# coecms/xmhw

Measured on AMD Instinct MI355X. Metric: grid-cells/sec for threshold() on 40yr daily SST, higher is better.
Workload: dtype f32 in / f64 out; 1 GPU; 0.25deg global (configs[2]): 1036800 cells per step, 1982-2021 (T=14610), windowHalfWidth=5, pctile=90, smoothPercentileWidth=31, nan_frac=0.0, skipna=False; cells_rank0=1036800, T=14610, D=366, kernel=clim_sorted_f32 (sorted row-lists in LDS, 2 lanes per cell, layout 40), slabs=1, gather=none

## Files before the change

xmhw_amd/csrc/kernels_sorted.hip:

```cpp
#include <type_traits>

#include "device_common.h"
#include "kernels.h"
#include "packed_src.h"
#include "plan.h"
#include "sortnet_gen.h"

namespace xmhw {
namespace {

typedef __attribute__((address_space(3))) uint32_t lds_u32;
__device__ __forceinline__ uint32_t lds_ld(uint32_t a) { return *reinterpret_cast<lds_u32*>(static_cast<uintptr_t>(a)); }
__device__ __forceinline__ void lds_st(uint32_t a, uint32_t v) { *reinterpret_cast<lds_u32*>(static_cast<uintptr_t>(a)) = v; }

constexpr int kSwap1 = 0xB1;
__device__ __forceinline__ uint32_t swp(uint32_t v) {
    return static_cast<uint32_t>(__builtin_amdgcn_update_dpp(0, static_cast<int>(v), kSwap1, 0xF, 0xF, true));
}
__device__ __forceinline__ double swp(double v) {
    const uint64_t b = static_cast<uint64_t>(__double_as_longlong(v));
    const uint32_t lo = swp(static_cast<uint32_t>(b)), hi = swp(static_cast<uint32_t>(b >> 32));
    return __longlong_as_double(static_cast<long long>((static_cast<uint64_t>(hi) << 32) | lo));
}
__device__ __forceinline__ uint32_t med3u(uint32_t a, uint32_t b, uint32_t c) {
    uint32_t r;
    asm("v_med3_u32 %0, %1, %2, %3" : "=v"(r) : "v"(a), "v"(b), "v"(c));
    return r;
}
__device__ __forceinline__ bool wave_any(bool c) { return __builtin_amdgcn_ballot_w64(c) != 0ull; }
__device__ __forceinline__ uint32_t mad_u24(uint32_t a, uint32_t b, uint32_t c) {
    uint32_t r;
    asm("v_mad_u32_u24 %0, %1, %2, %3" : "=v"(r) : "v"(a), "s"(b), "v"(c));
    return r;
}
__device__ __forceinline__ uint32_t mad_i24(uint32_t a, int32_t b, uint32_t c) {
    uint32_t r;
    asm("v_mad_i32_i24 %0, %1, %2, %3" : "=v"(r) : "v"(a), "v"(b), "v"(c));
    return r;
}
__device__ __forceinline__ uint32_t umin(uint32_t a, uint32_t b) { return a < b ? a : b; }
__device__ __forceinline__ uint32_t umax(uint32_t a, uint32_t b) { return a > b ? a : b; }

template <bool NEG>
__device__ __forceinline__ uint32_t key_fast(uint32_t b) {
    const int32_t sg = static_cast<int32_t>(b) >> 31;
    if constexpr (NEG)
        return static_cast<uint32_t>(__builtin_amdgcn_bitop3_b32(sg, static_cast<int32_t>(b), static_cast<int32_t>(0x80000000u), 0xC9));
    else
        return static_cast<uint32_t>(__builtin_amdgcn_bitop3_b32(sg, static_cast<int32_t>(b), static_cast<int32_t>(0x80000000u), 0x36));
}

__device__ __forceinline__ uint32_t count_ge4(uint32_t a0, uint32_t a1, uint32_t a2, uint32_t a3, uint32_t th) {
    uint32_t c;
    unsigned long long s0, s1, s2, s3, sd;
    asm("v_cmp_ge_u32_e64 %[s0], %[a0], %[t]\n\t"
        "v_cmp_ge_u32_e64 %[s1], %[a1], %[t]\n\t"
        "v_cmp_ge_u32_e64 %[s2], %[a2], %[t]\n\t"
        "v_cmp_ge_u32_e64 %[s3], %[a3], %[t]\n\t"
        "v_addc_co_u32_e64 %[c], %[sd], 0, 0, %[s0]\n\t"
        "v_addc_co_u32_e64 %[c], %[sd], %[c], 0, %[s1]\n\t"
        "v_addc_co_u32_e64 %[c], %[sd], %[c], 0, %[s2]\n\t"
        "v_addc_co_u32_e64 %[c], %[sd], %[c], 0, %[s3]"
        : [c] "=&v"(c), [s0] "=&s"(s0), [s1] "=&s"(s1), [s2] "=&s"(s2), [s3] "=&s"(s3), [sd] "=&s"(sd)
        : [a0] "v"(a0), [a1] "v"(a1), [a2] "v"(a2), [a3] "v"(a3), [t] "v"(th));
    return c;
}

typedef uint32_t V32 __attribute__((ext_vector_type(32)));
#ifdef XMHW_NO_COLD
#define XMHW_COLD(x) (x)
#else
#define XMHW_COLD(x) __builtin_expect(!!(x), 0)
#endif
#define XMHW_STR2(x) #x
#define XMHW_STR(x) XMHW_STR2(x)
#ifndef XMHW_LOOP_PAD
#define XMHW_LOOP_PAD 0
#endif

template <int N>
__device__ __forceinline__ void sort_desc(uint32_t (&v)[N]) {
    if constexpr (N >= 3 && N <= 7) {
        sortnet::Ins<N>::run(v);
    } else if constexpr (N == 8 || N == 10 || N == 12) {
        constexpr int H = N / 2;
        uint32_t a[H], b[H];
#pragma unroll
        for (int i = 0; i < H; ++i) { a[i] = v[i]; b[i] = v[H + i]; }
        sortnet::Ins<H>::run(a);
        sortnet::Ins<H>::run(b);
#pragma unroll
        for (int i = 0; i < H; ++i) { v[i] = a[i]; v[H + i] = b[i]; }
        sortnet::MergeTop<H, H, N>::run(v);
    } else {
        sortnet::Desc<N>::run(v);
    }
}
constexpr int kLdsGranule = 1280;


__device__ __forceinline__ uint32_t wave_min_u32(uint32_t v) {
    v = umin(v, static_cast<uint32_t>(__builtin_amdgcn_update_dpp(-1, static_cast<int>(v), 0xB1, 0xF, 0xF, false)));
    v = umin(v, static_cast<uint32_t>(__builtin_amdgcn_update_dpp(-1, static_cast<int>(v), 0x4E, 0xF, 0xF, false)));
    v = umin(v, static_cast<uint32_t>(__builtin_amdgcn_update_dpp(-1, static_cast<int>(v), 0x141, 0xF, 0xF, false)));
    v = umin(v, static_cast<uint32_t>(__builtin_amdgcn_update_dpp(-1, static_cast<int>(v), 0x140, 0xF, 0xF, false)));
    const uint32_t a = static_cast<uint32_t>(__builtin_amdgcn_readlane(static_cast<int>(v), 0));
    const uint32_t b = static_cast<uint32_t>(__builtin_amdgcn_readlane(static_cast<int>(v), 16));
    const uint32_t c = static_cast<uint32_t>(__builtin_amdgcn_readlane(static_cast<int>(v), 32));
    const uint32_t d = static_cast<uint32_t>(__builtin_amdgcn_readlane(static_cast<int>(v), 48));
    return umin(umin(a, b), umin(c, d));
}
__device__ __forceinline__ uint32_t wave_max_u32(uint32_t v) { return ~wave_min_u32(~v); }

template <int KPL>
__device__ __forceinline__ void pool_order_stats(const uint32_t (&key)[KPL], uint32_t n, uint32_t lo, uint32_t guess,
                                                 uint32_t& out_lo, uint32_t& out_hi) {
    auto count_lt = [&](uint32_t v) -> uint32_t {
        uint32_t cnt = 0;
#pragma unroll
        for (int i = 0; i < KPL; ++i)
            cnt += static_cast<uint32_t>(__builtin_popcountll(__builtin_amdgcn_ballot_w64(key[i] != 0u && key[i] < v)));
        return cnt;
    };
    auto count_eq = [&](uint32_t v) -> uint32_t {
        uint32_t cnt = 0;
#pragma unroll
        for (int i = 0; i < KPL; ++i)
            cnt += static_cast<uint32_t>(__builtin_popcountll(__builtin_amdgcn_ballot_w64(key[i] == v)));
        return cnt;
    };
    auto next_above = [&](uint32_t v) -> uint32_t {
        uint32_t m = 0xFFFFFFFFu;
#pragma unroll
        for (int i = 0; i < KPL; ++i) m = (key[i] > v && key[i] < m) ? key[i] : m;
        return wave_min_u32(m);
    };
    auto next_below = [&](uint32_t v) -> uint32_t {
        uint32_t m = 0;
#pragma unroll
        for (int i = 0; i < KPL; ++i) m = (key[i] < v && key[i] > m) ? key[i] : m;
        return wave_max_u32(m);
    };
    uint32_t v = guess;
    bool found = false;
    uint32_t cl = 0, ev = 0;
    if (v != 0u) {
        cl = count_lt(v);
        ev = count_eq(v);
        for (int it = 0; it < 32 && !found; ++it) {
            if (cl <= lo && lo < cl + ev) {
                found = true;
            } else if (lo < cl) {
                v = next_below(v);
                if (v == 0u) break;
                ev = count_eq(v);
                cl -= ev;
            } else {
                const uint32_t nv = next_above(v);
                if (nv == 0xFFFFFFFFu) break;
                cl += ev;
                v = nv;
                ev = count_eq(v);
            }
        }
    }
    if (!found) {
        v = 0;
        for (int bit = 31; bit >= 0; --bit) {
            const uint32_t cand = v | (1u << bit);
            uint32_t cnt = 0;
#pragma unroll
            for (int i = 0; i < KPL; ++i)
                cnt += static_cast<uint32_t>(__builtin_popcountll(__builtin_amdgcn_ballot_w64(key[i] - 1u < cand - 1u)));
            if (cnt <= lo) v = cand;
        }
        cl = count_lt(v);
        ev = count_eq(v);
    }
    uint32_t vhi = v;
    if (lo + 1 < n && lo + 1 >= cl + ev) vhi = next_above(v);
    out_lo = v;
    out_hi = vhi;
}

}

template <int YPS, int K, int KL, bool STATS, bool PACKED>
__device__ __forceinline__ void sorted_body(
    const void* __restrict__ ts, int64_t C, int64_t ld, int64_t Tn, const uint32_t* __restrict__ table,
    const uint32_t* __restrict__ sflags, const DevSortedChunk* __restrict__ chunks, double q, int negate,
    int32_t ntracks, double* __restrict__ thresh, double* __restrict__ seas, int64_t ldo,
    unsigned long long* __restrict__ stats, const PackedI16& pk) {
    constexpr int R = 11;
    constexpr uint32_t ES = PACKED ? 2u : 4u;
    constexpr int NL = 6;
    constexpr int HE = (YPS + 1) / 2 * 2;
    constexpr int HH = HE / 2;
    constexpr int KH = K / 2;
#ifndef XMHW_SERIAL_MAX
#define XMHW_SERIAL_MAX 3
#endif
    constexpr uint32_t kSerialMax = XMHW_SERIAL_MAX;
    constexpr int NTP = 2 * YPS;
    constexpr uint32_t LSTRIDE = 32 * 4;
    constexpr uint32_t RSTRIDE = R * LSTRIDE;
    constexpr int LDS_BYTES = (R * KL * static_cast<int>(LSTRIDE) + kLdsGranule - 1) / kLdsGranule * kLdsGranule;
    static_assert(K <= HE && K % 2 == 0, "a list stores an even number of keys, at most what a lane holds");
    constexpr int EXT = K - KL;
    static_assert(EXT == 0 || ((EXT == 2 || EXT == 4) && KL >= KH), "two or four register ranks, all from lane 1's half");
    constexpr int EXN = EXT > 0 ? EXT : 1;
    static_assert(LDS_BYTES == 8960 || LDS_BYTES == 11520 || LDS_BYTES == 14080 || LDS_BYTES == 17920 || LDS_BYTES == 20480 ||
                  LDS_BYTES == 23040 || LDS_BYTES == 25600, "sorted_lds_probe() checks these allocation sizes");
    __shared__ __attribute__((aligned(16))) uint32_t lds[LDS_BYTES / 4];

    const int lane = threadIdx.x & 63;
    const int sub = lane & 1;
    const int cw = lane >> 1;
    const int64_t cell = static_cast<int64_t>(blockIdx.x) * 32 + cw;
    const bool cell_ok = cell < C;
    const DevSortedChunk ch = chunks[blockIdx.y];
    const int32_t step_min = ch.warm_start - ch.trow0;
    const char* col = static_cast<const char*>(ts) + (cell_ok ? cell : C - 1) * static_cast<int64_t>(ES);
    const bool mirror = q < 0.5;
    const int kneg = (negate != 0) != mirror ? 1 : 0;
    const uint32_t tmax = static_cast<uint32_t>(Tn - 1);
    const bool padded_last = (YPS - 1) * 2 + sub >= ntracks;
    const uint32_t padmask = padded_last ? 0xFFFFFFFFu : 0u;
    const uint32_t* tab = table + sub;

    const uint32_t lds0 = static_cast<uint32_t>(reinterpret_cast<uintptr_t>((lds_u32*)lds));
    if (lds0 != 0u) __builtin_trap();
    const uint32_t lcell = static_cast<uint32_t>(cw) * 4u;
    for (int i = lane; i < LDS_BYTES / 4; i += 64) lds[i] = 0u;
    __builtin_amdgcn_s_waitcnt(0);
    __builtin_amdgcn_wave_barrier();

    uint32_t P[NL];
    V32 TV = 0;
#define XMHW_RSLO(j) TV[2 * (j)]
#define XMHW_RSHI(j) TV[2 * (j) + 1]
#define XMHW_EX(e, j) TV[12 + 6 * (e) + (j)]
#define XMHW_NVL(j) TV[24 + (j)]
    uint32_t lbase[NL];
#pragma unroll
    for (int j = 0; j < NL; ++j) {
        const int g = sub * NL + j;
        lbase[j] = g < R ? lcell + static_cast<uint32_t>(g) * LSTRIDE : 0x40000000u + lcell;
        P[j] = 0;
    }
    static_assert(KL >= 5, "a list holds a window");
    static_assert(NL == 6 && EXT <= 2, "the register vector holds five values of six lists");
#ifdef XMHW_WARM_SELECT
    uint32_t Ctop = 0, n = 0, B = 0u;
#else
    uint32_t Ctop = 0, n = 0, B = 0xFFFFFFFFu;
#endif
    double total = 0.0;

    const uint32_t ld4 = static_cast<uint32_t>(ld) * ES;
    const char* ap[YPS];
    auto entries_of = [&](int32_t step, uint32_t (&e)[YPS]) {
        const uint32_t* p = tab + static_cast<int64_t>(step - step_min) * NTP;
#pragma unroll
        for (int y = 0; y < YPS; ++y) e[y] = p[y * 2];
    };
    auto point_at = [&](int32_t step) {
        uint32_t e[YPS];
        entries_of(step, e);
#pragma unroll
        for (int y = 0; y < YPS; ++y) {
            const uint32_t t = umin((e[y] >> 1) - 2u, tmax);
            ap[y] = col + static_cast<uint64_t>(t) * ld4;
        }
    };
    auto advance = [&]() {
#pragma unroll
        for (int y = 0; y < YPS; ++y) ap[y] += (y == YPS - 1 && padded_last) ? 0u : ld4;
    };
    typename std::conditional<PACKED, int32_t, float>::type x_in[YPS];
    auto request = [&]() {
#pragma unroll
        for (int y = 0; y < YPS; ++y) {
            if constexpr (PACKED) x_in[y] = static_cast<int32_t>(*reinterpret_cast<const int16_t*>(ap[y]));
            else x_in[y] = *reinterpret_cast<const float*>(ap[y]);
        }
    };
    point_at(ch.warm_start);
    request();

    unsigned long long tacc[8] = {0, 0, 0, 0, 0, 0, 0, 0};
    unsigned long long tlast = 0;
    if constexpr (STATS) tlast = __builtin_amdgcn_s_memtime();
    auto tick = [&](int idx) {
        if constexpr (STATS) {
            __builtin_amdgcn_sched_barrier(0);
            asm volatile("s_waitcnt lgkmcnt(0)" ::: "memory");
            const unsigned long long now = __builtin_amdgcn_s_memtime();
            tacc[idx] += now - tlast;
            tlast = now;
            __builtin_amdgcn_sched_barrier(0);
        }
    };
    uint32_t st_rows = 0, st_iter = 0, st_flag = 0, st_steps = 0;
    uint32_t st_serial = 0, st_ext = 0;
    uint32_t st_more[4] = {0, 0, 0, 0};

    uint32_t e_alo = 0, e_ahi = 0, e_n = 0;
    double e_total = 0.0, e_g = 0.0;

    int32_t ep_s = -1;
    uint32_t ep_eph = 0;
    auto finish_rows = [&]() {
        double th = make_nan(), se = make_nan();
        if (e_n > 0) {
            double v_lo = static_cast<double>(key_f32(e_alo));
            double v_hi = static_cast<double>(key_f32(e_ahi));
            if (mirror) {
                v_lo = -v_lo;
                v_hi = -v_hi;
            }
            se = e_total / static_cast<double>(e_n);
            if constexpr (PACKED) {
                v_lo = packed_value(pk, v_lo);
                v_hi = packed_value(pk, v_hi);
                se = packed_value(pk, se);
            }
            th = numpy_lerp(v_lo, v_hi, e_g);
        }
        if (static_cast<uint32_t>(sub) <= ep_eph && cell_ok) {
            const int64_t row = static_cast<int64_t>(ep_s) - static_cast<int64_t>(ep_eph) + sub;
            thresh[row * ldo + cell] = th;
            seas[row * ldo + cell] = se;
        }
        ep_s = -1;
    };
    bool nan_mode = false;
    uint32_t vi_n = 0xFFFFFFFFu, vi_lo = 0;
    double vi_g = 0.0;
    int m = ((ch.warm_start % R) + R) % R;
    uint32_t sf_cur = __builtin_amdgcn_readfirstlane(sflags[ch.warm_start - step_min]);
    uint32_t sf_nxt = ch.warm_start + 1 < ch.end ? __builtin_amdgcn_readfirstlane(sflags[ch.warm_start + 1 - step_min]) : 0u;
#ifdef XMHW_LOOP_ALIGN
    asm volatile(".p2align " XMHW_STR(XMHW_LOOP_ALIGN) "\n\t.rept " XMHW_STR(XMHW_LOOP_PAD) "\n\ts_nop 0\n\t.endr" ::: "memory");
#endif
    for (int32_t s = ch.warm_start; s < ch.end; ++s) {
        const uint32_t sf = sf_cur;
        const uint32_t sf_nn = s + 2 < ch.end ? sflags[s + 2 - step_min] : 0u;
        uint32_t k[HE];
        double din = 0.0;
        uint32_t nvin = 0;
        float xv[YPS];
        bool packed_fill = false;
        if constexpr (STATS) {
            asm volatile("s_waitcnt vmcnt(0)" ::: "memory");
            tick(5);
        }
        if constexpr (PACKED) {
            if (pk.swap) {
#pragma unroll
                for (int y = 0; y < YPS; ++y)
                    x_in[y] = static_cast<int32_t>(static_cast<int16_t>(__builtin_bswap16(static_cast<uint16_t>(x_in[y]))));
            }
#pragma unroll
            for (int y = 0; y < YPS; ++y) xv[y] = static_cast<float>(x_in[y]);
            if (pk.mode == 1) {
#pragma unroll
                for (int y = 0; y < YPS; ++y) {
                    float f = xv[y] * pk.sf;
                    f = f + pk.of;
                    xv[y] = f;
                }
            }
            bool anyfill = false;
#pragma unroll
            for (int y = 0; y < YPS; ++y) anyfill = anyfill || x_in[y] == pk.fill;
            packed_fill = wave_any(anyfill);
            if (packed_fill) {
#pragma unroll
                for (int y = 0; y < YPS; ++y) xv[y] = x_in[y] == pk.fill ? __uint_as_float(0x7FC00000u) : xv[y];
            }
        } else {
#pragma unroll
            for (int y = 0; y < YPS; ++y) xv[y] = x_in[y];
        }
        bool slow = !(sf & 1u) || nan_mode;
        if (!slow) {
            auto plain_row = [&](auto negc, auto sumc) {
                constexpr bool NEG = decltype(negc)::value, SUM = decltype(sumc)::value;
                double din1 = 0.0;
#pragma unroll
                for (int y = 0; y < YPS; ++y) {
                    uint32_t xb = __float_as_uint(xv[y]);
                    uint32_t ky = key_fast<NEG>(xb);
                    if (y == YPS - 1) {
                        xb &= ~padmask;
                        ky &= ~padmask;
                    }
                    k[y] = ky;
                    if constexpr (SUM) {
                        const double dv = static_cast<double>(__uint_as_float(xb));
                        if (y & 1) din1 = y == 1 ? dv : din1 + dv;
                        else din = y == 0 ? dv : din + dv;
                    }
                }
                if constexpr (SUM) din += din1;
            };
            bool int_sum = false;
            if constexpr (PACKED) int_sum = pk.mode != 1;
            if (int_sum) {
                if constexpr (PACKED) {
                    int32_t isum = 0;
#pragma unroll
                    for (int y = 0; y < YPS; ++y)
                        isum += (y == YPS - 1) ? (x_in[y] & static_cast<int32_t>(~padmask)) : x_in[y];
                    if (kneg) plain_row(std::true_type{}, std::false_type{});
                    else plain_row(std::false_type{}, std::false_type{});
                    din = packed_fill ? make_nan() : static_cast<double>(isum);
                }
            } else if (kneg) {
                plain_row(std::true_type{}, std::true_type{});
            } else {
                plain_row(std::false_type{}, std::true_type{});
            }
            if (negate) din = -din;
            nvin = padded_last ? YPS - 1 : YPS;
            slow = wave_any(din != din);
            nan_mode = slow;
        }
        if (XMHW_COLD(slow)) {
            din = 0.0;
            nvin = 0;
#define XMHW_GENERAL_ROW(NEG_, OKEXPR)                                                                  \
    _Pragma("unroll") for (int y = 0; y < YPS; ++y) {                                                   \
        const float xs = xv[y];                                                                          \
        const bool ok = xs == xs && (OKEXPR);                                                            \
        k[y] = ok ? key_fast<NEG_>(__float_as_uint(xs)) : 0u;                                            \
        din += static_cast<double>(ok ? xs : 0.0f);                                                      \
        nvin += ok ? 1u : 0u;                                                                            \
    }
            if (sf & 1u) {
                if (kneg) { XMHW_GENERAL_ROW(true, !(y == YPS - 1 && padded_last)) }
                else { XMHW_GENERAL_ROW(false, !(y == YPS - 1 && padded_last)) }
            } else {
                uint32_t e[YPS];
                entries_of(s, e);
                if (kneg) { XMHW_GENERAL_ROW(true, (e[y] >> 1) >= 2u) }
                else { XMHW_GENERAL_ROW(false, (e[y] >> 1) >= 2u) }
            }
#undef XMHW_GENERAL_ROW
            if (negate) din = -din;
            if (sf & 1u) nan_mode = wave_any(nvin != static_cast<uint32_t>(padded_last ? YPS - 1 : YPS));
        }
#pragma unroll
        for (int y = YPS; y < HE; ++y) k[y] = 0u;
        tick(6);
        if (ep_s >= 0) finish_rows();
        if (s + 1 < ch.end) {
            if (!XMHW_COLD(!(sf_nxt & 2u))) advance();
            else point_at(s + 1);
            request();
        }
        tick(0);

        uint32_t u[KH];
        {
            uint32_t ka[HE];
            {
                uint32_t h0[HH], h1[HH];
#pragma unroll
                for (int i = 0; i < HH; ++i) { h0[i] = k[i]; h1[i] = k[HH + i]; }
                sort_desc<HH>(h0);
                sort_desc<HH>(h1);
#pragma unroll
                for (int i = 0; i < HH; ++i) { ka[i] = h0[i]; ka[HH + i] = h1[i]; }
            }
            sortnet::MergeTop<HH, HH, K>::run(ka);
            uint32_t t[K];
#pragma unroll
            for (int i = 0; i < K; ++i) t[i] = umax(ka[i], swp(ka[K - 1 - i]));
            const uint32_t lb = sub ? 0u : 0xFFFFFFFFu;
#pragma unroll
            for (int i = 0; i < KH; ++i) u[i] = med3u(t[i], t[i + KH], lb);
            sortnet::BitonicDesc<KH>::run(u);
        }
        tick(1);

        const int m_sub = m >= NL ? 1 : 0;
        const int mj = __builtin_amdgcn_readfirstlane(m - m_sub * NL);
        const bool own_m = sub == m_sub;
        const uint32_t base_m = lcell + static_cast<uint32_t>(m) * LSTRIDE + static_cast<uint32_t>(sub * KH) * RSTRIDE;
#pragma unroll
        for (int i = 0; i < KH; ++i) {
            if (EXT == 0 || i < KH - EXT || sub == 0) lds_st(base_m + static_cast<uint32_t>(i) * RSTRIDE, u[i]);
        }
        uint32_t c_old = 0, nv_old = 0;
        bool is_slot[NL];
#pragma unroll
        for (int j = 0; j < NL; ++j) {
            int mj_ = mj;
            asm volatile("" : "+s"(mj_));
            is_slot[j] = mj_ == j;
        }
        const uint32_t nvm = TV[24 + mj];
        {
            uint32_t Pm = P[0];
#pragma unroll
            for (int j = 1; j < NL; ++j) Pm = is_slot[j] ? P[j] : Pm;
            if (own_m) {
                c_old = Pm;
                nv_old = nvm;
            }
        }
        uint32_t c_new = 0;
#pragma unroll
        for (int i = 0; i < KH; ++i) c_new += (u[i] > B) ? 1u : 0u;
        {
            uint32_t pk = (c_new << 16) | nvin;
            uint32_t po = (c_old << 16) | nv_old;
            pk += swp(pk);
            po += swp(po);
            c_new = umin(pk >> 16, static_cast<uint32_t>(KL));
            nvin = pk & 0xFFFFu;
            c_old = po >> 16;
            nv_old = po & 0xFFFFu;
        }
        din += swp(din);
        Ctop += c_new - c_old;
        n += nvin - nv_old;
#pragma unroll
        for (int j = 0; j < NL; ++j) P[j] = (own_m && is_slot[j]) ? c_new : P[j];
        TV[24 + mj] = own_m ? nvin : nvm;
        if constexpr (EXT > 0) {
#pragma unroll
            for (int e_ = 0; e_ < EXT; ++e_) {
                const uint32_t r_ = swp(u[KH - EXT + e_]);
                const uint32_t mine = sub ? u[KH - EXT + e_] : r_;
                const uint32_t old_ = TV[12 + 6 * e_ + mj];
                TV[12 + 6 * e_ + mj] = own_m ? mine : old_;
            }
        }
        {
            const uint64_t db = static_cast<uint64_t>(__double_as_longlong(din));
            const uint32_t ol_ = TV[2 * mj], oh_ = TV[2 * mj + 1];
            TV[2 * mj] = own_m ? static_cast<uint32_t>(db) : ol_;
            TV[2 * mj + 1] = own_m ? static_cast<uint32_t>(db >> 32) : oh_;
        }
        {
            double tsum = 0.0;
#pragma unroll
            for (int j = 0; j < NL; ++j)
                tsum += __longlong_as_double(static_cast<long long>((static_cast<uint64_t>(XMHW_RSHI(j)) << 32) | XMHW_RSLO(j)));
            total = tsum + swp(tsum);
        }
        m = (m + 1 == R) ? 0 : m + 1;
        tick(2);

        uint32_t a_lo = 0, a_hi = 0;
        double g = 0.0;
        bool flag = false;
#ifdef XMHW_WARM_SELECT
        if (true) {
#else
        if (s >= ch.begin) {
#endif
        if (XMHW_COLD(wave_any(n != vi_n))) {
            vi_n = n;
            const uint32_t nn_ = n ? n : 1u;
            const double vi = static_cast<double>(nn_ - 1) * q;
            const double fl = floor(vi);
            vi_g = vi - fl;
            vi_lo = static_cast<uint32_t>(fl);
        }
        const uint32_t nn = n ? n : 1u;
        g = vi_g;
        const uint32_t lo = vi_lo;
        const bool need2 = lo + 1 < nn;
        const uint32_t Cs = n ? (mirror ? lo + 1u : n - 1u - lo) : 0u;
        const bool grow = Ctop <= Cs;
        uint32_t rem = grow ? Cs - Ctop : Ctop - Cs;
        const uint32_t steps0 = rem;
        const uint32_t cm = grow ? 0u : 0xFFFFFFFFu;
        const uint32_t cneg = grow ? 0u : 1u;
        auto cpl = [&](uint32_t v) -> uint32_t { return (v ^ cm) + cneg; };
        const int psign = grow ? 1 : -1;
        const int32_t dstep = grow ? static_cast<int32_t>(RSTRIDE) : -static_cast<int32_t>(RSTRIDE);
        uint32_t wbase[NL];
#pragma unroll
        for (int j = 0; j < NL; ++j) wbase[j] = lbase[j] - (grow ? 0u : RSTRIDE);
        uint32_t prem = rem;
        uint32_t st_iter_row = 0;
        bool st_first_done = false;
        bool first_round = true;
        while (wave_any(prem != 0u)) {
            if (XMHW_COLD(!first_round && !wave_any(prem > kSerialMax))) {
                while (wave_any(prem != 0u)) {
                    if constexpr (STATS) ++st_serial;
                    uint32_t hd[NL];
                    uint32_t hm = 0;
#pragma unroll
                    for (int j = 0; j < NL; ++j) {
                        hd[j] = cpl(lds_ld(mad_u24(P[j], RSTRIDE, wbase[j])));
                        hm = umax(hm, hd[j]);
                    }
                    const uint32_t ho = swp(hm);
                    const uint32_t cmax = umax(hm, ho);
                    const bool act = prem != 0u;
                    const bool dry_ = act && cmax == 0u;
                    const bool win = act && !dry_ && hm == cmax && (sub == 0 || ho != cmax);
                    bool found = false;
#pragma unroll
                    for (int j = 0; j < NL; ++j) {
                        const bool sel = win && !found && hd[j] == cmax;
                        P[j] += sel ? static_cast<uint32_t>(psign) : 0u;
                        found = found || sel;
                    }
                    rem -= (act && !dry_) ? 1u : 0u;
                    flag = flag | dry_;
                    prem = flag ? 0u : rem;
                }
                break;
            }
            first_round = false;
            if constexpr (STATS) {
                ++st_iter;
#if defined(XMHW_HIST_W3)
                if (false) {
#elif defined(XMHW_HIST_FIRST)
                if (!st_first_done) {
#else
                if (st_first_done) {
#endif
                    uint32_t r_ = prem;
#pragma unroll
                    for (int off = 32; off >= 1; off >>= 1) r_ = umax(r_, static_cast<uint32_t>(__shfl_xor(static_cast<int>(r_), off, 64)));
                    #ifdef XMHW_HIST_FIRST
                    ++st_more[r_ <= XMHW_H1 ? 1 : r_ <= XMHW_H2 ? 2 : 3];
#else
                    ++st_more[r_ <= 2u ? 0 : r_ <= 4u ? 1 : r_ <= 8u ? 2 : 3];
#endif
                }
                st_first_done = true;
            }
            const uint32_t d = umin(prem, 15u);
            uint32_t a[NL][4];
            uint32_t F = 0;
            {
                uint32_t ad[NL][5];
#pragma unroll
                for (int j = 0; j < NL; ++j) {
                    ad[j][0] = mad_u24(P[j], RSTRIDE, wbase[j]);
#pragma unroll
                    for (int i = 1; i < 5; ++i) ad[j][i] = ad[j][i - 1] + static_cast<uint32_t>(dstep);
                }
                __builtin_amdgcn_sched_barrier(0);
                uint32_t raw[NL][5];
#pragma unroll
                for (int j = 0; j < NL; ++j)
#pragma unroll
                    for (int i = 0; i < 5; ++i) raw[j][i] = lds_ld(ad[j][i]);
                __builtin_amdgcn_sched_barrier(0);
#pragma unroll
                for (int j = 0; j < NL; ++j) {
#pragma unroll
                    for (int i = 0; i < 4; ++i) a[j][i] = cpl(raw[j][i]);
                    F = umax(F, cpl(raw[j][4]));
                }
            }
#ifndef XMHW_LANE_TOP
#define XMHW_LANE_TOP 16
#endif
            constexpr int LT = XMHW_LANE_TOP;
            static_assert(LT == 12 || LT == 16, "merge networks exist for these");
            uint32_t sl[LT];
            {
                uint32_t r01[8], r23[8], r45[8];
#pragma unroll
                for (int i = 0; i < 4; ++i) {
                    r01[i] = a[0][i]; r01[4 + i] = a[1][i];
                    r23[i] = a[2][i]; r23[4 + i] = a[3][i];
                    r45[i] = a[4][i]; r45[4 + i] = a[5][i];
                }
                sortnet::MergeTop<4, 4, 8>::run(r01);
                sortnet::MergeTop<4, 4, 8>::run(r23);
                sortnet::MergeTop<4, 4, 8>::run(r45);
                uint32_t r4[16];
#pragma unroll
                for (int i = 0; i < 8; ++i) { r4[i] = r01[i]; r4[8 + i] = r23[i]; }
                sortnet::MergeTop<8, 8, LT>::run(r4);
                uint32_t r6[LT + 8];
#pragma unroll
                for (int i = 0; i < LT; ++i) r6[i] = r4[i];
#pragma unroll
                for (int i = 0; i < 8; ++i) r6[LT + i] = r45[i];
                sortnet::MergeTop<LT, 8, LT>::run(r6);
#pragma unroll
                for (int i = 0; i < LT; ++i) sl[i] = r6[i];
            }
            if constexpr (LT < 16) F = umax(F, sl[LT - 1]);
            uint32_t u8[8];
            {
                uint32_t t16[16];
#pragma unroll
                for (int i = 0; i < 16; ++i) {
                    if (i < LT && 15 - i < LT) t16[i] = umax(sl[i], swp(sl[15 - i]));
                    else if (i < LT) t16[i] = sl[i];
                    else t16[i] = swp(sl[15 - i]);
                }
                const uint32_t lb = sub ? 0u : 0xFFFFFFFFu;
#pragma unroll
                for (int i = 0; i < 8; ++i) u8[i] = med3u(t16[i], t16[i + 8], lb);
            }
            uint32_t tl;
            {
                const uint32_t idx = (d - 1u) - (sub ? 8u : 0u);
                const int32_t nidx = static_cast<int32_t>(~idx);
                const uint32_t b4 = static_cast<uint32_t>(__builtin_amdgcn_sbfe(nidx, 2, 1));
                const uint32_t b2 = static_cast<uint32_t>(__builtin_amdgcn_sbfe(nidx, 1, 1));
                const uint32_t b1 = static_cast<uint32_t>(__builtin_amdgcn_sbfe(nidx, 0, 1));
                const uint32_t c0 = med3u(u8[0], u8[4], b4), c1 = med3u(u8[1], u8[5], b4);
                const uint32_t c2 = med3u(u8[2], u8[6], b4), c3 = med3u(u8[3], u8[7], b4);
                const uint32_t e0 = med3u(c0, c2, b2), e1 = med3u(c1, c3, b2);
                uint32_t z = med3u(e0, e1, b1);
                z = idx < 8u ? z : 0u;
                tl = z | swp(z);
            }
            F = umax(F, swp(F));
            const bool act = d != 0u;
            const bool unsafe = act && tl < F;
            const bool dry = act && !unsafe && tl == 0u;
            const bool move = act && !dry;
            const uint32_t th = move ? (unsafe ? F : tl) : 0xFFFFFFFFu;
#ifdef XMHW_HIST_W3
            if constexpr (STATS) {
                if (st_iter_row == 0) {
                    uint32_t f3 = 0;
#pragma unroll
                    for (int j = 0; j < NL; ++j) f3 = umax(f3, a[j][3]);
                    f3 = umax(f3, swp(f3));
                    ++st_more[wave_any(act && tl < f3) ? 2 : 1];
                }
                ++st_iter_row;
            }
#endif
            uint32_t pj[NL];
            uint32_t psum = 0;
#pragma unroll
            for (int j = 0; j < NL; ++j) {
                pj[j] = count_ge4(a[j][0], a[j][1], a[j][2], a[j][3], th);
                psum += pj[j];
            }
            uint32_t moved = psum + swp(psum);
            const bool tie = move & !unsafe & (moved > d);
            if (XMHW_COLD(wave_any(tie))) {
                asm volatile("" ::: "memory");
                uint32_t gj[NL];
                uint32_t gsum = 0;
#pragma unroll
                for (int j = 0; j < NL; ++j) {
                    gj[j] = count_ge4(a[j][0], a[j][1], a[j][2], a[j][3], tl + 1u);
                    gsum += gj[j];
                }
                const uint32_t G = gsum + swp(gsum);
                const uint32_t e_mine = psum - gsum;
                const uint32_t e_other = swp(e_mine);
                int32_t room = static_cast<int32_t>(d - G) - static_cast<int32_t>(sub ? e_other : 0u);
                uint32_t ps2 = 0;
#pragma unroll
                for (int j = 0; j < NL; ++j) {
                    const int32_t ej = static_cast<int32_t>(pj[j] - gj[j]);
                    const int32_t take = room < 0 ? 0 : (room < ej ? room : ej);
                    room -= ej;
                    const uint32_t pt = gj[j] + static_cast<uint32_t>(take);
                    pj[j] = tie ? pt : pj[j];
                    ps2 += pt;
                }
                psum = tie ? ps2 : psum;
                moved = psum + swp(psum);
            }
#pragma unroll
            for (int j = 0; j < NL; ++j) P[j] = mad_i24(pj[j], psign, P[j]);
            rem -= moved;
            flag = flag | dry;
            prem = flag ? 0u : rem;
        }
        {
            uint32_t ao[NL], ai[NL], ho[NL], hi_[NL];
#pragma unroll
            for (int j = 0; j < NL; ++j) {
                ao[j] = mad_u24(P[j], RSTRIDE, lbase[j]);
                ai[j] = ao[j] - RSTRIDE;
            }
            __builtin_amdgcn_sched_barrier(0);
#pragma unroll
            for (int j = 0; j < NL; ++j) {
                ho[j] = lds_ld(ao[j]);
                hi_[j] = lds_ld(ai[j]);
            }
            __builtin_amdgcn_sched_barrier(0);
            uint32_t mx = 0, mn = 0xFFFFFFFFu;
#pragma unroll
            for (int j = 0; j < NL; ++j) {
                mx = umax(mx, ho[j]);
                mn = umin(mn, hi_[j] - 1u);
            }
            a_lo = umax(mx, swp(mx));
            a_hi = umin(mn, swp(mn)) + 1u;
        }
        Ctop = mad_i24(rem, -psign, Cs);
        if (!need2) {
            if (mirror) a_lo = a_hi;
            else a_hi = a_lo;
        }
        if constexpr (EXT > 0) {
            bool anyx = false;
#pragma unroll
            for (int j = 0; j < NL; ++j) anyx = anyx | ((P[j] == static_cast<uint32_t>(KL)) & (XMHW_EX(0, j) > a_lo));
            if (XMHW_COLD(wave_any(anyx & !flag))) {
                asm volatile("" ::: "memory");
                uint32_t pv[NL];
                uint32_t need = 0;
#pragma unroll
                for (int j = 0; j < NL; ++j) {
                    const bool sat = (P[j] == static_cast<uint32_t>(KL)) & !flag;
                    uint32_t c_ = 0;
#pragma unroll
                    for (int e_ = 0; e_ < EXT; ++e_) c_ += XMHW_EX(e_, j) > a_lo ? 1u : 0u;
                    pv[j] = sat ? c_ : 0u;
                    need += pv[j];
                }
                need += swp(need);
                if constexpr (STATS) ++st_ext;
                const bool fix = need != 0u;
                auto heads = [&](uint32_t (&hd)[NL]) -> uint32_t {
                    uint32_t lv[NL];
#pragma unroll
                    for (int j = 0; j < NL; ++j) lv[j] = lds_ld(lbase[j] + (P[j] - 1u) * RSTRIDE);
                    uint32_t hm = 0xFFFFFFFFu;
#pragma unroll
                    for (int j = 0; j < NL; ++j) {
                        uint32_t ev = XMHW_EX(0, j);
#pragma unroll
                        for (int e_ = 1; e_ < EXT; ++e_) ev = pv[j] > static_cast<uint32_t>(e_) ? XMHW_EX(e_, j) : ev;
                        hd[j] = (pv[j] != 0u ? ev : lv[j]) - 1u;
                        hm = umin(hm, hd[j]);
                    }
                    return hm;
                };
                uint32_t vlast = a_lo;
                while (wave_any(need != 0u)) {
                    uint32_t hd[NL];
                    const uint32_t hm = heads(hd);
                    const uint32_t ho = swp(hm);
                    const uint32_t cmin = umin(hm, ho);
                    const bool act = need != 0u;
                    const bool win = act && hm == cmin && (sub == 0 || ho != cmin);
                    bool found = false;
#pragma unroll
                    for (int j = 0; j < NL; ++j) {
                        const bool sel = win && !found && hd[j] == cmin;
                        const bool reg = pv[j] != 0u;
                        P[j] = (sel && !reg) ? P[j] - 1u : P[j];
                        pv[j] = (sel && reg) ? pv[j] - 1u : pv[j];
                        found = found || sel;
                    }
                    if (act) {
                        vlast = cmin + 1u;
                        need -= 1u;
                    }
                }
                uint32_t hd[NL];
                uint32_t hm = heads(hd);
                hm = umin(hm, swp(hm)) + 1u;
                uint32_t pvs = 0;
#pragma unroll
                for (int j = 0; j < NL; ++j) pvs += pv[j];
                pvs += swp(pvs);
                if (fix) {
                    a_lo = vlast;
                    a_hi = hm;
                    if (!need2) {
                        if (mirror) a_lo = a_hi;
                        else a_hi = a_lo;
                    }
                    Ctop = Cs - pvs;
#pragma unroll
                    for (int j = 0; j < NL; ++j) flag = flag || (pv[j] == static_cast<uint32_t>(EXT) && XMHW_NVL(j) > static_cast<uint32_t>(K));
                }
            }
        } else {
            uint32_t atb = 0;
#pragma unroll
            for (int j = 0; j < NL; ++j)
                atb |= (P[j] == static_cast<uint32_t>(K) && XMHW_NVL(j) > static_cast<uint32_t>(K)) ? (1u << j) : 0u;
            if (XMHW_COLD(wave_any(atb != 0u))) {
#pragma unroll
                for (int j = 0; j < NL; ++j) {
                    const uint32_t Uj = lds_ld(lbase[j] + static_cast<uint32_t>(K - 1) * RSTRIDE);
                    flag = flag || (((atb >> j) & 1u) && Uj > a_lo);
                }
            }
        }
        B = a_lo;
        {
            const uint32_t fl_ = flag ? 1u : 0u;
            flag = (fl_ | swp(fl_)) != 0u;
        }
        if constexpr (STATS) st_flag += (sub == 0 && cell_ok && flag) ? 1u : 0u;
        tick(3);
        if (XMHW_COLD(s >= ch.begin && wave_any(flag))) {
            constexpr int KPL = (NTP * R + 63) / 64;
            unsigned long long fm = __builtin_amdgcn_ballot_w64(flag && sub == 0 && cell_ok);
            while (fm != 0ull) {
                const int L = __builtin_ctzll(fm);
                fm &= fm - 1ull;
                const int64_t cc = static_cast<int64_t>(blockIdx.x) * 32 + (L >> 1);
                const uint32_t n_c = static_cast<uint32_t>(__builtin_amdgcn_readlane(static_cast<int>(n), L));
                uint32_t lo_c = static_cast<uint32_t>(__builtin_amdgcn_readlane(static_cast<int>(lo), L));
                if (mirror) lo_c = lo_c + 1u < n_c ? n_c - 2u - lo_c : 0u;
                const uint32_t guess = static_cast<uint32_t>(__builtin_amdgcn_readlane(static_cast<int>(a_lo), L));
                uint32_t key[KPL];
                {
                    uint32_t ent[KPL];
#pragma unroll
                    for (int i = 0; i < KPL; ++i) {
                        const int e = lane + 64 * i;
                        const int j = e / NTP, trk = e - j * NTP;
                        ent[i] = e < NTP * R ? table[static_cast<int64_t>(s - j - step_min) * NTP + trk] : (kCodeInvalid << 1);
                    }
                    const char* colc = static_cast<const char*>(ts) + cc * static_cast<int64_t>(ES);
                    typename std::conditional<PACKED, int32_t, float>::type raw[KPL];
#pragma unroll
                    for (int i = 0; i < KPL; ++i) {
                        const uint32_t t = umin((ent[i] >> 1) - 2u, tmax);
                        const char* a_ = colc + static_cast<uint64_t>(t) * ld4;
                        if constexpr (PACKED) raw[i] = static_cast<int32_t>(*reinterpret_cast<const int16_t*>(a_));
                        else raw[i] = *reinterpret_cast<const float*>(a_);
                    }
#pragma unroll
                    for (int i = 0; i < KPL; ++i) {
                        float xs;
                        if constexpr (PACKED) {
                            int32_t c_ = raw[i];
                            if (pk.swap) c_ = static_cast<int32_t>(static_cast<int16_t>(__builtin_bswap16(static_cast<uint16_t>(c_))));
                            xs = packed_sample(pk, c_);
                        } else {
                            xs = raw[i];
                        }
                        const bool ok = xs == xs && (ent[i] >> 1) >= 2u;
                        const uint32_t kk = kneg ? key_fast<true>(__float_as_uint(xs)) : key_fast<false>(__float_as_uint(xs));
                        key[i] = ok ? kk : 0u;
                    }
                }
                uint32_t r_lo = 0, r_hi = 0;
                pool_order_stats<KPL>(key, n_c, lo_c, guess, r_lo, r_hi);
                const bool mine = (lane >> 1) == (L >> 1);
                if (mirror && !(lo_c + 1u < n_c && n_c >= 2u)) r_hi = r_lo;
                a_lo = mine ? r_lo : a_lo;
                a_hi = mine ? r_hi : a_hi;
                flag = mine ? false : flag;
            }
        }
        tick(7);
        if constexpr (STATS) st_steps += (sub == 0 && cell_ok) ? steps0 : 0u;
        }
        tick(3);

        if (s >= ch.begin) {
            if constexpr (STATS) ++st_rows;
            const uint32_t eph = static_cast<uint32_t>(s - ch.begin) & 1u;
            if (static_cast<uint32_t>(sub) == eph) {
                e_alo = mirror ? a_hi : a_lo;
                e_ahi = mirror ? a_lo : a_hi;
                e_n = n;
                e_total = total;
                e_g = g;
            }
            if (eph == 1u || s + 1 == ch.end) {
                ep_s = s;
                ep_eph = eph;
            }
        }
        tick(4);
        sf_cur = sf_nxt;
        sf_nxt = __builtin_amdgcn_readfirstlane(sf_nn);
    }
    if (ep_s >= 0) finish_rows();
    if (STATS && stats != nullptr) {
        if (lane == 0) {
            atomicAdd(&stats[0], static_cast<unsigned long long>(st_rows));
            atomicAdd(&stats[1], static_cast<unsigned long long>(st_iter));
#pragma unroll
            for (int i = 1; i < 4; ++i) atomicAdd(&stats[4 + i], static_cast<unsigned long long>(st_more[i]));
            atomicAdd(&stats[4], static_cast<unsigned long long>(st_ext));
#pragma unroll
            for (int i = 0; i < 8; ++i) atomicAdd(&stats[8 + i], tacc[i]);
        }
        if (sub == 0) {
            atomicAdd(&stats[2], static_cast<unsigned long long>(st_flag));
            atomicAdd(&stats[3], static_cast<unsigned long long>(st_steps));
        }
    }
}

#ifndef XMHW_WAVES3_MAX_YPS
#define XMHW_WAVES3_MAX_YPS 8
#endif
#define XMHW_WAVES_PER_SIMD(Y) ((Y) <= XMHW_WAVES3_MAX_YPS ? 3 : 2)
template <int YPS, int K, int KL, bool STATS>
__global__ __launch_bounds__(64, XMHW_WAVES_PER_SIMD(YPS)) void clim_sorted_f32(
    const float* __restrict__ ts, int64_t C, int64_t ld, int64_t Tn, const uint32_t* __restrict__ table,
    const uint32_t* __restrict__ sflags, const DevSortedChunk* __restrict__ chunks, double q, int negate,
    int32_t ntracks, double* __restrict__ thresh, double* __restrict__ seas, int64_t ldo,
    unsigned long long* __restrict__ stats) {
    sorted_body<YPS, K, KL, STATS, false>(ts, C, ld, Tn, table, sflags, chunks, q, negate, ntracks, thresh, seas, ldo, stats,
                                      PackedI16{});
}
template <int YPS, int K, int KL>
__global__ __launch_bounds__(64, XMHW_WAVES_PER_SIMD(YPS)) void clim_sorted_i16(
    const int16_t* __restrict__ codes, PackedI16 pk, int64_t C, int64_t ld, int64_t Tn, const uint32_t* __restrict__ table,
    const uint32_t* __restrict__ sflags, const DevSortedChunk* __restrict__ chunks, double q, int negate,
    int32_t ntracks, double* __restrict__ thresh, double* __restrict__ seas, int64_t ldo) {
    sorted_body<YPS, K, KL, false, true>(codes, C, ld, Tn, table, sflags, chunks, q, negate, ntracks, thresh, seas, ldo, nullptr, pk);
}

namespace {
typedef void (*SortedKernel)(const float*, int64_t, int64_t, int64_t, const uint32_t*, const uint32_t*,
                             const DevSortedChunk*, double, int, int32_t, double*, double*, int64_t, unsigned long long*);
typedef void (*SortedKernelI16)(const int16_t*, PackedI16, int64_t, int64_t, int64_t, const uint32_t*, const uint32_t*,
                                const DevSortedChunk*, double, int, int32_t, double*, double*, int64_t);
struct SortedEntry { int yps, k, kl; SortedKernel fn, fn_stats; SortedKernelI16 fn_i16; };
#ifdef XMHW_RING_STATS
#define XMHW_SS(Y, K, KL) clim_sorted_f32<Y, K, KL, true>
#else
#define XMHW_SS(Y, K, KL) nullptr
#endif
#define XMHW_S2(Y, K, KL) {Y, K, KL, clim_sorted_f32<Y, K, KL, false>, XMHW_SS(Y, K, KL), clim_sorted_i16<Y, K, KL>}
#define XMHW_S(Y, K) XMHW_S2(Y, K, K)
#ifndef XMHW_K40
#define XMHW_K40 16
#endif
#ifndef XMHW_KL48
#define XMHW_KL48 16
#endif
#ifndef XMHW_KL40
#define XMHW_KL40 14
#endif
const SortedEntry kSorted[] = {
#ifdef XMHW_SORTED_ONLY
    XMHW_S2(20, XMHW_K40, XMHW_KL40),
#else
    XMHW_S(5, 6),   XMHW_S(6, 6),   XMHW_S(7, 8),   XMHW_S(8, 8),   XMHW_S(9, 10),  XMHW_S(10, 10), XMHW_S(11, 10),
    XMHW_S(12, 10), XMHW_S(13, 12), XMHW_S(14, 12), XMHW_S(15, 12), XMHW_S(16, 12), XMHW_S(17, 14), XMHW_S(18, 14),
    XMHW_S2(19, XMHW_K40, XMHW_KL40), XMHW_S2(20, XMHW_K40, XMHW_KL40), XMHW_S2(21, 18, XMHW_KL48), XMHW_S2(22, 18, XMHW_KL48), XMHW_S2(23, 18, XMHW_KL48), XMHW_S2(24, 18, XMHW_KL48),
#endif
};
#undef XMHW_S
#undef XMHW_S2
#undef XMHW_SS
const SortedEntry* find_sorted(int32_t yps) {
    for (const auto& e : kSorted)
        if (e.yps == yps) return &e;
    return nullptr;
}
}

namespace {
__global__ __launch_bounds__(64) void lds_outside_probe(uint32_t* __restrict__ bad, int BYTES) {
    extern __shared__ __attribute__((aligned(16))) uint32_t lds[];
    for (int i = threadIdx.x; i < BYTES / 4; i += 64) lds[i] = 0x80000000u | (blockIdx.x << 16) | static_cast<uint32_t>(i);
    __builtin_amdgcn_s_waitcnt(0);
    __builtin_amdgcn_wave_barrier();
    const uint32_t base = static_cast<uint32_t>(reinterpret_cast<uintptr_t>((lds_u32*)lds));
    uint32_t wrong = base != 0u ? 1u : 0u;
    const uint32_t lane4 = threadIdx.x * 4u;
    constexpr uint32_t RS = 11u * 128u;
    for (uint32_t r = 0; r < 6; ++r) {
        for (uint32_t gofs = 0; gofs + 256u <= 10u * 128u; gofs += 256u) {
            wrong |= lds_ld(static_cast<uint32_t>(BYTES) + r * RS + gofs + lane4);
            wrong |= lds_ld(0u - (r + 1u) * RS + gofs + lane4);
        }
        wrong |= lds_ld(0x40000000u + r * RS + lane4);
        wrong |= lds_ld(0x40000000u - (r + 1u) * RS + lane4);
    }
    if (lds_ld(static_cast<uint32_t>(BYTES) - 256u + lane4) != (0x80000000u | (blockIdx.x << 16) | static_cast<uint32_t>(BYTES / 4 - 64 + threadIdx.x)))
        wrong = 1u;
    if (wrong != 0u) atomicAdd(bad, 1u);
}
}

hipError_t sorted_lds_probe(uint32_t* d_bad, hipStream_t stream) {
    hipError_t e = hipMemsetAsync(d_bad, 0, sizeof(uint32_t), stream);
    if (e != hipSuccess) return e;
    for (int bytes : {8960, 11520, 14080, 17920, 20480, 23040, 25600})
        hipLaunchKernelGGL(lds_outside_probe, dim3(2048), dim3(64), static_cast<size_t>(bytes), stream, d_bad, bytes);
    return hipGetLastError();
}

int32_t sorted_pick_yps(int32_t w, int32_t ntracks) {
    if (w != 5) return 0;
    const int32_t yps = (ntracks + 1) / 2;
    return find_sorted(yps) ? yps : 0;
}

int32_t sorted_pick_k(int32_t w, int32_t ntracks) {
    if (w != 5) return 0;
    const SortedEntry* e = find_sorted((ntracks + 1) / 2);
    return e ? e->k : 0;
}

int32_t sorted_lds_bytes(int32_t w, int32_t ntracks) {
    if (w != 5) return 0;
    const SortedEntry* e = find_sorted((ntracks + 1) / 2);
    return e ? (11 * e->kl * 128 + kLdsGranule - 1) / kLdsGranule * kLdsGranule : 0;
}

hipError_t launch_sorted_f32(const float* ts, int64_t C, int64_t ld, int64_t Tn, const uint32_t* table,
                             const uint32_t* sflags, const DevSortedChunk* chunks, int32_t nchunks,
                             int32_t w, int32_t yps, int32_t ntracks, double q, int negate, double* thresh, double* seas,
                             int64_t ldo, hipStream_t stream, unsigned long long* stats) {
    const SortedEntry* e = w == 5 ? find_sorted(yps) : nullptr;
    if (!e || ld >= (int64_t(1) << 30)) return hipErrorInvalidValue;
    if (C <= 0 || nchunks <= 0) return hipSuccess;
    dim3 grid(static_cast<unsigned>((C + 31) / 32), static_cast<unsigned>(nchunks));
    const bool twin = stats != nullptr && e->fn_stats != nullptr;
    hipLaunchKernelGGL(twin ? e->fn_stats : e->fn, grid, dim3(64), 0, stream, ts, C, ld, Tn, table, sflags, chunks, q,
                       negate, ntracks, thresh, seas, ldo, twin ? stats : nullptr);
    return hipGetLastError();
}

hipError_t launch_sorted_i16(const int16_t* codes, const PackedI16& pk, int64_t C, int64_t ld, int64_t Tn,
                             const uint32_t* table, const uint32_t* sflags, const DevSortedChunk* chunks, int32_t nchunks,
                             int32_t w, int32_t yps, int32_t ntracks, double q, int negate, double* thresh, double* seas,
                             int64_t ldo, hipStream_t stream) {
    const SortedEntry* e = w == 5 ? find_sorted(yps) : nullptr;
    if (!e || !e->fn_i16 || ld >= (int64_t(1) << 30) || pk.mode < 1 || pk.mode > 3) return hipErrorInvalidValue;
    if (C <= 0 || nchunks <= 0) return hipSuccess;
    dim3 grid(static_cast<unsigned>((C + 31) / 32), static_cast<unsigned>(nchunks));
    hipLaunchKernelGGL(e->fn_i16, grid, dim3(64), 0, stream, codes, pk, C, ld, Tn, table, sflags, chunks, q, negate, ntracks,
                       thresh, seas, ldo);
    return hipGetLastError();
}

}
```

Measured before the change: 42.35 million cells/s.

## Defer flagged-cell fallback exact threshold into batched pending drain

```diff
diff --git a/xmhw_amd/csrc/kernels_sorted.hip b/xmhw_amd/csrc/kernels_sorted.hip
--- a/xmhw_amd/csrc/kernels_sorted.hip
+++ b/xmhw_amd/csrc/kernels_sorted.hip
@@ -76,6 +76,9 @@
 #define XMHW_STR(x) XMHW_STR2(x)
 #ifndef XMHW_LOOP_PAD
 #define XMHW_LOOP_PAD 0
+#endif
+#ifndef XMHW_DRAIN_BATCH
+#define XMHW_DRAIN_BATCH 4
 #endif
 
 template <int N>
@@ -307,6 +310,7 @@
 
     uint32_t e_alo = 0, e_ahi = 0, e_n = 0;
     double e_total = 0.0, e_g = 0.0;
+    bool e_def = false;
 
     int32_t ep_s = -1;
     uint32_t ep_eph = 0;
@@ -329,10 +333,130 @@
         }
         if (static_cast<uint32_t>(sub) <= ep_eph && cell_ok) {
             const int64_t row = static_cast<int64_t>(ep_s) - static_cast<int64_t>(ep_eph) + sub;
-            thresh[row * ldo + cell] = th;
+            if (!e_def) thresh[row * ldo + cell] = th;
             seas[row * ldo + cell] = se;
         }
         ep_s = -1;
+    };
+    constexpr int kPendCap = 64;
+    constexpr int kDrainBatch = XMHW_DRAIN_BATCH;
+    constexpr bool kDefer = YPS > 8;
+    static_assert(NTP * R < 1024, "the pool size of an item has ten bits");
+    uint32_t pd_meta = 0, pd_key = 0;
+    int32_t pd_n = 0;
+    auto drain_pending = [&]() {
+        constexpr int KPL = (NTP * R + 63) / 64;
+        if constexpr (!STATS) {
+            if (stats != nullptr && lane == 0) atomicAdd(&stats[2], static_cast<unsigned long long>(pd_n));
+        }
+        for (int32_t i0 = 0; i0 < pd_n; i0 += kDrainBatch) {
+            uint32_t meta[kDrainBatch], guess[kDrainBatch];
+#pragma unroll
+            for (int b = 0; b < kDrainBatch; ++b) {
+                const int32_t ix = i0 + b < pd_n ? i0 + b : pd_n - 1;
+                meta[b] = static_cast<uint32_t>(__builtin_amdgcn_readlane(static_cast<int>(pd_meta), ix));
+                guess[b] = static_cast<uint32_t>(__builtin_amdgcn_readlane(static_cast<int>(pd_key), ix));
+            }
+            uint32_t ent[kDrainBatch][KPL];
+            uint32_t eoff[KPL];
+#pragma unroll
+            for (int i = 0; i < KPL; ++i) {
+                const int e = lane + 64 * i;
+                const int ec = e < NTP * R ? e : NTP * R - 1;
+                const int jc = ec / NTP, tc = ec - jc * NTP;
+                eoff[i] = static_cast<uint32_t>((R - 1 - jc) * NTP + tc);
+            }
+#pragma unroll
+            for (int b = 0; b < kDrainBatch; ++b) {
+                const int32_t sb = static_cast<int32_t>(meta[b] >> 16);
+                const uint32_t* rowp = table + static_cast<int64_t>(sb - (R - 1) - step_min) * NTP;
+#pragma unroll
+                for (int i = 0; i < KPL; ++i) {
+                    const uint32_t en = rowp[eoff[i]];
+                    ent[b][i] = lane + 64 * i < NTP * R ? en : (kCodeInvalid << 1);
+                }
+            }
+            typename std::conditional<PACKED, int32_t, float>::type raw[kDrainBatch][KPL];
+            uint32_t okm[kDrainBatch];
+#pragma unroll
+            for (int b = 0; b < kDrainBatch; ++b) {
+                const int64_t cc = static_cast<int64_t>(blockIdx.x) * 32 + static_cast<int64_t>(meta[b] & 31u);
+                const char* colc = static_cast<const char*>(ts) + cc * static_cast<int64_t>(ES);
+                okm[b] = 0u;
+#pragma unroll
+                for (int i = 0; i < KPL; ++i) {
+                    const uint32_t t = umin((ent[b][i] >> 1) - 2u, tmax);
+                    okm[b] |= (ent[b][i] >> 1) >= 2u ? (1u << i) : 0u;
+                    const char* a_ = colc + static_cast<uint64_t>(t) * ld4;
+                    if constexpr (PACKED) raw[b][i] = static_cast<int32_t>(*reinterpret_cast<const int16_t*>(a_));
+                    else raw[b][i] = *reinterpret_cast<const float*>(a_);
+                }
+            }
+            __builtin_amdgcn_s_waitcnt(0x0F70);
+            double th_out = make_nan();
+            int64_t at_out = 0;
+            for (int32_t b = 0; b < kDrainBatch && i0 + b < pd_n; ++b) {
+                typename std::conditional<PACKED, int32_t, float>::type rw[KPL];
+                uint32_t ok_b = okm[0], meta_b = meta[0], guess_b = guess[0];
+#pragma unroll
+                for (int i = 0; i < KPL; ++i) rw[i] = raw[0][i];
+#pragma unroll
+                for (int bb = 1; bb < kDrainBatch; ++bb) {
+                    if (b == bb) {
+                        ok_b = okm[bb];
+                        meta_b = meta[bb];
+                        guess_b = guess[bb];
+#pragma unroll
+                        for (int i = 0; i < KPL; ++i) rw[i] = raw[bb][i];
+                    }
+                }
+                uint32_t key[KPL];
+#pragma unroll
+                for (int i = 0; i < KPL; ++i) {
+                    float xs;
+                    if constexpr (PACKED) {
+                        int32_t c_ = rw[i];
+                        if (pk.swap) c_ = static_cast<int32_t>(static_cast<int16_t>(__builtin_bswap16(static_cast<uint16_t>(c_))));
+                        xs = packed_sample(pk, c_);
+                    } else {
+                        xs = rw[i];
+                    }
+                    const bool ok = xs == xs && ((ok_b >> i) & 1u) != 0u;
+                    const uint32_t kk = kneg ? key_fast<true>(__float_as_uint(xs)) : key_fast<false>(__float_as_uint(xs));
+                    key[i] = ok ? kk : 0u;
+                }
+                const uint32_t n_c = (meta_b >> 5) & 1023u;
+                const uint32_t nn_ = n_c ? n_c : 1u;
+                const double vi = static_cast<double>(nn_ - 1) * q;
+                const double fl = floor(vi);
+                const double g_c = vi - fl;
+                uint32_t lo_c = static_cast<uint32_t>(fl);
+                if (mirror) lo_c = lo_c + 1u < n_c ? n_c - 2u - lo_c : 0u;
+                uint32_t r_lo = 0, r_hi = 0;
+                pool_order_stats<KPL>(key, n_c, lo_c, guess_b, r_lo, r_hi);
+                if (mirror && !(lo_c + 1u < n_c && n_c >= 2u)) r_hi = r_lo;
+                double th = make_nan();
+                if (n_c > 0) {
+                    double v_lo = static_cast<double>(key_f32(mirror ? r_hi : r_lo));
+                    double v_hi = static_cast<double>(key_f32(mirror ? r_lo : r_hi));
+                    if (mirror) {
+                        v_lo = -v_lo;
+                        v_hi = -v_hi;
+                    }
+                    if constexpr (PACKED) {
+                        v_lo = packed_value(pk, v_lo);
+                        v_hi = packed_value(pk, v_hi);
+                    }
+                    th = numpy_lerp(v_lo, v_hi, g_c);
+                }
+                const int64_t at = static_cast<int64_t>(meta_b >> 16) * ldo + static_cast<int64_t>(blockIdx.x) * 32 +
+                                   static_cast<int64_t>(meta_b & 31u);
+                th_out = lane == b ? th : th_out;
+                at_out = lane == b ? at : at_out;
+            }
+            if (lane < kDrainBatch && i0 + lane < pd_n) thresh[at_out] = th_out;
+        }
+        pd_n = 0;
     };
     bool nan_mode = false;
     uint32_t vi_n = 0xFFFFFFFFu, vi_lo = 0;
@@ -444,6 +568,7 @@
             } else {
                 uint32_t e[YPS];
                 entries_of(s, e);
+                __builtin_amdgcn_s_waitcnt(0x0F70);
                 if (kneg) { XMHW_GENERAL_ROW(true, (e[y] >> 1) >= 2u) }
                 else { XMHW_GENERAL_ROW(false, (e[y] >> 1) >= 2u) }
             }
@@ -907,7 +1032,19 @@
         }
         if constexpr (STATS) st_flag += (sub == 0 && cell_ok && flag) ? 1u : 0u;
         tick(3);
-        if (XMHW_COLD(s >= ch.begin && wave_any(flag))) {
+        if (kDefer && XMHW_COLD(s >= ch.begin && wave_any(flag))) {
+            unsigned long long fm = __builtin_amdgcn_ballot_w64(flag && sub == 0 && cell_ok);
+            const uint32_t it_meta = static_cast<uint32_t>(cw) | (n << 5) | (static_cast<uint32_t>(s) << 16);
+            while (fm != 0ull) {
+                const int L = __builtin_ctzll(fm);
+                fm &= fm - 1ull;
+                pd_meta = lane == pd_n ? static_cast<uint32_t>(__builtin_amdgcn_readlane(static_cast<int>(it_meta), L)) : pd_meta;
+                pd_key = lane == pd_n ? static_cast<uint32_t>(__builtin_amdgcn_readlane(static_cast<int>(a_lo), L)) : pd_key;
+                ++pd_n;
+            }
+        }
+        if (kDefer && XMHW_COLD(pd_n > kPendCap - 32 || (s + 1 == ch.end && pd_n != 0))) drain_pending();
+        if (!kDefer && XMHW_COLD(s >= ch.begin && wave_any(flag))) {
             constexpr int KPL = (NTP * R + 63) / 64;
             unsigned long long fm = __builtin_amdgcn_ballot_w64(flag && sub == 0 && cell_ok);
             while (fm != 0ull) {
@@ -974,6 +1111,7 @@
                 e_n = n;
                 e_total = total;
                 e_g = g;
+                if constexpr (kDefer) e_def = flag;
             }
             if (eph == 1u || s + 1 == ch.end) {
                 ep_s = s;
@@ -1047,7 +1185,11 @@
 #endif
 const SortedEntry kSorted[] = {
 #ifdef XMHW_SORTED_ONLY
+#ifdef XMHW_ONLY_SHORT
+    XMHW_S(8, 8),
+#else
     XMHW_S2(20, XMHW_K40, XMHW_KL40),
+#endif
 #else
     XMHW_S(5, 6),   XMHW_S(6, 6),   XMHW_S(7, 8),   XMHW_S(8, 8),   XMHW_S(9, 10),  XMHW_S(10, 10), XMHW_S(11, 10),
     XMHW_S(12, 10), XMHW_S(13, 12), XMHW_S(14, 12), XMHW_S(15, 12), XMHW_S(16, 12), XMHW_S(17, 14), XMHW_S(18, 14),
@@ -1124,7 +1266,7 @@
     dim3 grid(static_cast<unsigned>((C + 31) / 32), static_cast<unsigned>(nchunks));
     const bool twin = stats != nullptr && e->fn_stats != nullptr;
     hipLaunchKernelGGL(twin ? e->fn_stats : e->fn, grid, dim3(64), 0, stream, ts, C, ld, Tn, table, sflags, chunks, q,
-                       negate, ntracks, thresh, seas, ldo, twin ? stats : nullptr);
+                       negate, ntracks, thresh, seas, ldo, stats);
     return hipGetLastError();
 }
 
```

Measured after the change: 41.18 million cells/s. 2.8% lower.
